# medical-genomics-group/sgVAMP-py

Measured on AMD Instinct MI355X. Metric: VAMP iterations/sec (and effective LD-matvec GB/s) at M markers, K cohorts, higher is better.
Workload: dtype f64

## Files before the change

include/sgvamp_hip.h:

```cpp
#ifndef SGVAMP_HIP_H
#define SGVAMP_HIP_H

#include <stdint.h>

#ifdef __cplusplus
extern "C" {
#endif

#define SGV_OK 0
#define SGV_ERR_HIP (-1)
#define SGV_ERR_ARG (-2)
#define SGV_ERR_RCCL (-3)
#define SGV_ERR_STATE (-4)

#define SGV_ABI_VERSION 2
int sgv_abi_version(void);

#define SGV_MAX_COHORTS 1024
#define SGV_MAX_SLABS 8

#define SGV_VEC_R 0
#define SGV_VEC_R1 1
#define SGV_VEC_XHAT1 2
#define SGV_VEC_XHAT2 3
// ... 132 lines not shown
int sgv_outputs_wait(sgv_ctx* ctx, int slot, double** data);

int sgv_lmmse(sgv_ctx* ctx, int it, const double* gamw, const double* gam2,
              const double* alpha1, const double* alpha2_prev, const int8_t* probes,
              int cg_maxit, double rtol, int lmmse_damp, double rho, int learn_gamw,
              double* out, int* cg_out, int* ld_passes_out);

int sgv_metrics(sgv_ctx* ctx, double* out4);
int sgv_metrics_begin(sgv_ctx* ctx);
int sgv_metrics_end(sgv_ctx* ctx, double* out4);


int sgv_ld_matvec(sgv_ctx* ctx, int ld, int ncol, const double* v, double* y);

int sgv_ld_pass_ex(sgv_ctx* ctx, int ld, int ncol, const double* in, const double* c1,
                   const double* c2, const double* w, uint32_t dot_mask, uint32_t yout_mask,
                   double ys1, double ys0, int run, double* out, double* yout, double* dots);

int sgv_cg_solve(sgv_ctx* ctx, int ld, int ncol, const double* c1, const double* c2,
                 const double* b, double* x, int maxiter, double rtol, int* iters_out,
                 int* info_out);

#define SGV_TIMERS_N 10
int sgv_timers(sgv_ctx* ctx, double* t, int cap, int reset);
#define SGV_EXCHANGE_STATS_N 16
int sgv_exchange_stats(sgv_ctx* ctx, double* out, int cap, int reset);

#define SGV_COMM_INFO_N 5
int sgv_comm_info(sgv_ctx* ctx, int* out, int cap, char* pci_bus_id, int pci_len);

int sgv_exchange_probe(sgv_ctx* ctx, int reps, double* us_out);

int sgv_em_cost_model(double cohort_markers, int nranks, double latency_us, double steps,
                      double* out2);

#define SGV_KIND_NONE 0
#define SGV_KIND_VALU 1
#define SGV_KIND_STRIP4 2
#define SGV_KIND_PAIR 3
#define SGV_KIND_WIDE 4
#define SGV_KIND_STRIP16 5
#define SGV_KIND_WALK 6
#define SGV_PF_KIND 0
#define SGV_PF_VALU_CLASS 1
#define SGV_PF_REST_KIND 2
#define SGV_PF_LOAD_FORM 3
#define SGV_PF_FIN_FORM 4
#define SGV_PF_PK_WIDTH 5
#define SGV_PF_PK_PAIRED 6
#define SGV_PF_DENSE 7
#define SGV_PF_SIDE 8
#define SGV_PF_REST_SIDE 9
#define SGV_PF_MFMA16 10
#define SGV_PF_IDLE_EXIT 11
#define SGV_PF_N 12
int sgv_ld_pass_form(sgv_ctx* ctx, int ld, int ncol, int32_t* form, int cap);

#define SGV_PS_BITS 0
#define SGV_PS_DENSE 1
#define SGV_PS_PACKED 2
#define SGV_PS_WALKS 3
#define SGV_PS_WIDE 4
#define SGV_PS_REST 5
#define SGV_PS_RAGGED 6
#define SGV_PS_PAIR 7
#define SGV_PS_REST_RAGGED 8
#define SGV_PS_REST_PAIR 9
#define SGV_PS_WIDE_IDLE 10
#define SGV_PS_NGRP 11
#define SGV_PS_WIDE_NGRP 12
#define SGV_PS_REST_NGRP 13
#define SGV_PS_N 14
#define SGV_SW_BAND_WALK 0
#define SGV_SW_F32_WALK 1
#define SGV_SW_MF_WIDE 2
#define SGV_SW_MF_PAIR 3
#define SGV_SW_MF_WIDE_IDLE 4
#define SGV_SW_F32_FORM 5
#define SGV_SW_FIN_FORM 6
#define SGV_SW_N 7
int sgv_pass_form_model(const int32_t* shape, const int32_t* switches, int mfma_min, int ncol,
                        int32_t* form, int cap);

int sgv_sync(sgv_ctx* ctx);

int sgv_read_bw(sgv_ctx* ctx, int64_t bytes, int reps, double* gbps);

#ifdef __cplusplus
}
#endif
#endif
```

sgvamp-py_amd/csrc/ctx.h:

```cpp
#pragma once
#include "common.h"
#include "hybrd.h"
#include "../../include/sgvamp_hip.h"

#include <rccl/rccl.h>

#include <algorithm>
#include <atomic>
#include <chrono>
#include <condition_variable>
#include <functional>
#include <mutex>
#include <thread>
#include <limits>
#include <cmath>
#include <cstdarg>
#include <cstdio>
#include <cstdlib>
#include <cstring>
#include <string>
#include <utility>
#include <vector>

using namespace sgv;
// ... 3 lines not shown
  int bits = 64;
  float* f32() const { return reinterpret_cast<float*>(ptr); }
  size_t esz() const { return bits == 32 ? sizeof(float) : sizeof(double); }
  int64_t ext = 0;
  std::vector<int64_t> poff, pw;
  int64_t* d_poff = nullptr;
  int64_t* d_pw = nullptr;
  double stored_bytes = 0.0;
  double stored_elems = 0.0;
};

struct LdCoupling {
  int gb = -1, nr = 0, nc = 0;
  double* d_up = nullptr;
  double* d_lo = nullptr;
};

struct GenoBlock {
  uint32_t* d_bits = nullptr;
  double* d_lut = nullptr;
  double* d_msd = nullptr;
  int64_t stride_w = 0;
  int nsamp = 0;
  int64_t nbad = 0;
};

struct StripSet {
  SymStrip* d_strips = nullptr;
  SymItem* d_sitems = nullptr;
  SymPanel* d_panels = nullptr;
  SymPanelW* d_wpanels = nullptr;
  int nstrips = 0, npanels = 0, nsitems = 0;
  int nslots_items = 0;
  bool ragged = false;
  int pair = 0;
  int ngrp = 1;
  std::vector<int> gs, gp;
};

struct LdPlan {
  bool valid = false;
  int bits = 64;
  RowGroup* d_rg = nullptr;
  int nrg = 0;
  int* d_pbeg = nullptr;
  int nparts = 0;
  SymItem* d_items[4] = {nullptr, nullptr, nullptr, nullptr};
  int nitems[4] = {0, 0, 0, 0};
  SymPanel* d_panels[4] = {nullptr, nullptr, nullptr, nullptr};
  int npanels = 0;
  StripSet s512;
  StripSet wide, rest;
  bool wide_idle = true;
  SymWalk* d_walks = nullptr;
  int nwalks = 0;
  SymPanel* d_wpanels = nullptr;
  SymItem* d_witems = nullptr;
  WalkFin* d_wfins = nullptr;
  int nwfins = 0, nhslots = 0, ncslots = 0;
  double stored_bytes = 0.0, dense_bytes = 0.0;
  double mac_elems = 0.0;
  CouplingTask* d_ctasks = nullptr;
  int nctasks = 0, ncp = 0;
  bool halo = false;
  int64_t hmax = 0, h_src0 = 0, h_src1 = 0;
  int h_len0 = 0, h_len1 = 0;
  double cpl_bytes = 0.0;
};

static inline int mfma_min_default() { return 3; }
static inline int cg_pipe_default() {
  const char* e = ab_env("SGV_CG_PIPE");
  return (e && e[0] == '0') ? 0 : 1;
}
constexpr int CG_RING = 4;
constexpr int MAXGRP = 8;
constexpr int NOUT_SLOTS = 3;

static inline int cg_exact_default() {
  const char* e = ab_env("SGV_CG_EXACT");
  return !e ? -1 : (e[0] == '0' ? 0 : 1);
}
constexpr double CG_EXACT_MIN_BYTES = 24e9;
static inline int sym_class_nc(int cls) { return std::min(16, 2 << (cls + 1)); }

static inline bool fused_ctl_pays(int nv, int nblk) {
  return nblk <= EM_CTL_MAXBLK && nv * nblk <= 128;
}

struct sgv_ctx {
  int dev = 0;
  hipStream_t st = nullptr;
  int K = 0, nld = 0;
  std::vector<int> ld_of;
  int nblk = 0;
  std::vector<int64_t> bn, boff, bvoff;
  int64_t Mloc = 0, Mpad = 0;
  int blk0 = 0, nblk_global = 0;
  int64_t Mtot = 0;
  double s = 0.0;
  std::vector<double> Ncoh;
  std::vector<std::vector<LdBlock>> ldb;
  std::vector<int64_t> lda;
  std::vector<BlkDesc*> d_blks;
  std::vector<LdPlan> plan;
  std::vector<std::vector<LdCoupling>> cpl;
  std::vector<GenoBlock> geno;
  std::vector<int> rank_blk0;
  double* d_cpbuf = nullptr;
  size_t cpbuf_cap = 0;
  double* d_halo = nullptr;
  size_t halo_cap = 0;
  double* h_halo = nullptr;
  size_t h_halo_cap = 0;
  int packing = 1;
  int ld_bits = 64;
  hipStream_t st_fin = nullptr;
  hipEvent_t ev_grp[MAXGRP] = {};
  hipEvent_t ev_fin = nullptr;
  double* d_whead = nullptr;
  double* d_wcarry = nullptr;
  size_t whead_cap = 0, wcarry_cap = 0;
  double* d_rowpart = nullptr;
  double* d_colpart = nullptr;
  size_t rowpart_cap = 0, colpart_cap = 0, part_cap = 0;
  int mfma_min = 3;
  double* d_pk = nullptr;
  double* d_out = nullptr;
  double* h_out[NOUT_SLOTS] = {};
  hipEvent_t ev_out[NOUT_SLOTS] = {};
  int8_t* h_probe[2] = {nullptr, nullptr};
  hipEvent_t ev_probe[2] = {nullptr, nullptr};
  int8_t* d_probe = nullptr;
  std::atomic<size_t> probe_cap{0};
  std::atomic<int> probe_slot{0};
  hipEvent_t ev_unpk[2] = {nullptr, nullptr};
  int pref_slot = -1;
  const int8_t* pref_src = nullptr;
  hipStream_t st_copy = nullptr;
  hipEvent_t ev_pack[NOUT_SLOTS] = {};
  double* h_met = nullptr;
  hipEvent_t ev_met = nullptr;
  int met_pending = 0;
  std::thread worker;
  std::mutex wmu;
  std::condition_variable wcv;
  struct Job {
    std::function<int()> fn;
    std::atomic<int> state{0};
    int rc = 0;
  };
  Job jobs[2];
  uint64_t job_begun = 0, job_ended = 0, job_run = 0;
  std::atomic<bool> worker_quit{false};
  struct Chain {
    int valid = 0;
    std::vector<double> gam1, gamw, alpha1, alpha2;
    double lam, om[MAXL];
  } chain;
  double mle_gam = std::numeric_limits<double>::quiet_NaN();
  double* d_inner = nullptr;
  size_t inner_cap = 0;
  int post_on = 0;
  double post_thr = 0.95;
  double* d_post = nullptr;
  size_t post_cap = 0;
// ... 157 lines not shown
```

sgvamp-py_amd/csrc/ldplan.hip:

```cpp
#include "ctx.h"

void free_plan(LdPlan& p){
  if (p.d_rg) (void)hipFree(p.d_rg);
  if (p.d_pbeg) (void)hipFree(p.d_pbeg);
  for (int k = 0; k < 4; ++k) {
    if (p.d_items[k]) (void)hipFree(p.d_items[k]);
    if (p.d_panels[k]) (void)hipFree(p.d_panels[k]);
  }
  for (StripSet* q : {&p.s512, &p.wide, &p.rest}) {
    if (q->d_strips) (void)hipFree(q->d_strips);
    if (q->d_sitems) (void)hipFree(q->d_sitems);
    if (q->d_panels) (void)hipFree(q->d_panels);
    if (q->d_wpanels) (void)hipFree(q->d_wpanels);
  }
  if (p.d_ctasks) (void)hipFree(p.d_ctasks);
  if (p.d_walks) (void)hipFree(p.d_walks);
  if (p.d_wpanels) (void)hipFree(p.d_wpanels);
  if (p.d_witems) (void)hipFree(p.d_witems);
  if (p.d_wfins) (void)hipFree(p.d_wfins);
  p = LdPlan();
}

void free_block(LdBlock& lb){
  if (lb.ptr) (void)hipFree(lb.ptr);
// ... 2 lines not shown
  lb = LdBlock();
}

static int64_t panel_ext(int64_t n, int64_t r0, int64_t ext) {
  return ext > 0 ? std::min(n - r0, ext) : n - r0;
}

int ld_alloc(sgv_ctx* c, int ld, int b, int fmt, int64_t ext){
  LdBlock& lb = c->ldb[ld][b];
  if (fmt == 0) ext = 0;
  const int bits = fmt == 1 ? c->ld_bits : 64;
  if (lb.ptr && lb.fmt == fmt && lb.ext == ext && lb.bits == bits) return SGV_OK;
  free_block(lb);
  c->plan[ld].valid = false;
  const int64_t n = c->bn[b];
  size_t elems = 0;
  lb.fmt = fmt;
  lb.ext = ext;
  lb.bits = bits;
  if (fmt == 0) {
    elems = (size_t)c->lda[b] * (size_t)n;
    lb.stored_elems = (double)n * (double)n;
    lb.stored_bytes = lb.stored_elems * 8.0;
  } else {
    double valid = 0.0;
    for (int64_t r0 = 0; r0 < n; r0 += SYM_H) {
      const int64_t H = std::min<int64_t>(SYM_H, n - r0);
      const int64_t e = panel_ext(n, r0, ext);
      const int64_t w = round_up(e, PADV);
      lb.poff.push_back((int64_t)elems);
      lb.pw.push_back(w);
      elems += (size_t)(H * w);
      valid += (double)H * (double)e;
    }
    lb.stored_elems = valid;
    lb.stored_bytes = valid * (double)lb.esz();
    HIPCHK(hipMalloc(&lb.d_poff, sizeof(int64_t) * lb.poff.size()));
    HIPCHK(hipMalloc(&lb.d_pw, sizeof(int64_t) * lb.pw.size()));
    HIPCHK(hipMemcpy(lb.d_poff, lb.poff.data(), sizeof(int64_t) * lb.poff.size(),
                     hipMemcpyHostToDevice));
    HIPCHK(hipMemcpy(lb.d_pw, lb.pw.data(), sizeof(int64_t) * lb.pw.size(), hipMemcpyHostToDevice));
  }
  {
    const hipError_t e = hipMalloc(&lb.ptr, lb.esz() * elems);
    if (e != hipSuccess) {
      lb.ptr = nullptr;
      size_t fr = 0, tot = 0;
      (void)hipGetLastError();
      (void)hipMemGetInfo(&fr, &tot);
      return fail(c, SGV_ERR_HIP,
                  "LD matrix %d block %d (n=%lld, %s, %s): %.2f GB of device memory needed, "
                  "%.2f GB free: %s", ld, b, (long long)n,
                  fmt == 0 ? "dense" : ext > 0 ? "packed band" : "packed triangle",
                  bits == 32 ? "f32" : "f64", (double)lb.esz() * (double)elems / 1e9, (double)fr / 1e9,
                  hipGetErrorString(e));
    }
  }
  HIPCHK(hipMemsetAsync(lb.ptr, 0, lb.esz() * elems, c->st));
  BlkDesc d{fmt == 0 ? lb.ptr : nullptr, c->lda[b], c->bn[b], c->bvoff[b]};
  HIPCHK(hipMemcpyAsync(c->d_blks[ld] + b, &d, sizeof d, hipMemcpyHostToDevice, c->st));
  CHK(stream_wait(c));
  return SGV_OK;
}

static int ld_ready(sgv_ctx* c, int ld) {
  for (int b = 0; b < c->nblk; ++b)
    if (!c->ldb[ld][b].ptr)
      return fail(c, SGV_ERR_STATE, "LD matrix %d block %d has not been set", ld, b);
  return SGV_OK;
}

int grow(sgv_ctx* c, double** buf, size_t* cap, size_t need){
  if (need <= *cap) return SGV_OK;
  if (*buf) HIPCHK(hipFree(*buf));
  *buf = nullptr;
  HIPCHK(hipMalloc(buf, sizeof(double) * need));
  *cap = need;
  return SGV_OK;
}


constexpr int MFMA_STRIP = 8;

static int pass_groups(int nstrips, int nblk, int slots) {
  const int g = nstrips / std::max(1, 4 * slots);
  return std::max(1, std::min(std::min(g, 8), nblk));
}

static int device_cus() {
  int dev = 0, ncu = 256;
  if (hipGetDevice(&dev) == hipSuccess) {
    hipDeviceProp_t prop;
    if (hipGetDeviceProperties(&prop, dev) == hipSuccess && prop.multiProcessorCount > 0)
      ncu = prop.multiProcessorCount;
  }
  return ncu;
}

static double lpt_efficiency(std::vector<double> cost, int slots) {
  std::sort(cost.begin(), cost.end(), std::greater<double>());
  std::vector<double> load((size_t)slots, 0.0);
  double tot = 0.0;
  for (double x : cost) {
    auto it = std::min_element(load.begin(), load.end());
    *it += x;
    tot += x;
  }
  const double mk = *std::max_element(load.begin(), load.end());
  return mk > 0.0 ? tot / slots / mk : 1.0;
}

static int mfma_pair_choice(const std::vector<SymStrip>& strips,
                            const std::vector<SymItem>& sitems, int forced) {
  if (forced >= 0) return forced;
  const int ncu = device_cus();
  std::vector<double> cost;
  cost.reserve(strips.size());
  for (const SymStrip& st : strips) {
    double x = 0.0;
    for (int i = 0; i < st.npan; ++i) x += (double)sitems[st.it0 + i].H / SYM_H;
    cost.push_back(x * (double)st.ncmax / 512.0);
  }
  const double quad = lpt_efficiency(cost, 2 * ncu);
  const double pair = lpt_efficiency(cost, ncu);
  return pair >= quad + 0.03 ? 1 : 0;
}

static int build_strips(sgv_ctx* c, int ld, const std::vector<SymItem>& items,
                        const std::vector<SymPanel>& panels, bool wide, int which,
                        int pair_forced, StripSet* out) {
  const int cw = wide ? MFW_CW : 512;
  const int S = MFMA_STRIP;
  const int NPAR = cw / SYM_H;
  auto taken = [&](int b) {
    const LdBlock& lb = c->ldb[ld][b];
    return lb.fmt == 1 && (which == 0 || (which == 1) == (lb.ext == 0));
  };
  std::vector<SymItem> sitems;
  std::vector<SymStrip> strips;
  std::vector<int> sblk;
  std::vector<SymPanelW> sp;
  std::vector<int> pblk;
  int bp0 = 0;
  for (int b = 0; b < c->nblk; ++b) {
    if (c->ldb[ld][b].fmt != 1) continue;
    const int64_t n = c->bn[b];
    const int np = (int)c->ldb[ld][b].poff.size();
    if (!taken(b)) {
      bp0 += np;
      continue;
    }
    const int sp0 = (int)sp.size();
    for (int g = 0; g < np; ++g) {
      SymPanelW w;
      w.p = panels[bp0 + g];
      for (int k = 0; k < 4; ++k) w.sb[k] = w.se[k] = 0;
      sp.push_back(w);
      pblk.push_back(b);
    }
    for (int p = 0; p < NPAR; ++p)
      for (int64_t c0 = (int64_t)SYM_H * p; c0 < n; c0 += cw) {
        const int G = (int)(c0 / SYM_H);
        const int sb = (int)strips.size();
        const int64_t ext = c->ldb[ld][b].ext;
        const int glo = ext > 0 ? std::max(p, G - NPAR * (((int)(ext / SYM_H) - 1) / NPAR)) : p;
        for (int g0 = glo; g0 <= G; g0 += NPAR * S) {
          SymStrip st;
          st.it0 = (int)sitems.size();
          st.npan = 0;
          st.slot = (int)strips.size();
          st.ncmax = 0;
          for (int g = g0; g <= G && g < g0 + NPAR * S; g += NPAR) {
            const SymPanel& pn = panels[bp0 + g];
            const int idx = pn.item_begin + (int)((c0 - (int64_t)SYM_H * g) / cw);
            if (idx >= pn.item_end || items[idx].c0 != c0)
              return fail(c, SGV_ERR_STATE, "strip plan: item (%d, %lld) missing", g,
                          (long long)c0);
            sitems.push_back(items[idx]);
            st.ncmax = std::max(st.ncmax, items[idx].nc);
            ++st.npan;
          }
          strips.push_back(st);
          sblk.push_back(b);
        }
        for (int k = 0; k < NPAR; ++k)
          if (G + k < np) {
            sp[sp0 + G + k].sb[k] = sb;
            sp[sp0 + G + k].se[k] = (int)strips.size();
          }
      }
    bp0 += np;
  }
  *out = StripSet();
  out->nslots_items = (int)items.size();
  if (strips.empty()) return SGV_OK;
  const int ncu = device_cus();
  std::vector<int> grp(c->nblk, 0);
  int ngrp = pass_groups((int)strips.size(), c->nblk, wide ? ncu : 2 * ncu);
  {
    auto bytes = [&](int b) { return which == 0 || taken(b) ? c->ldb[ld][b].stored_bytes : 0.0; };
    double tot = 0.0;
    for (int b = 0; b < c->nblk; ++b) tot += bytes(b);
    double acc = 0.0;
    for (int b = 0; b < c->nblk; ++b) {
      grp[b] = std::min(ngrp - 1, (int)(acc / tot * ngrp));
      acc += bytes(b);
    }
    ngrp = grp[c->nblk - 1] + 1;
  }
  {
    std::vector<int> ord(strips.size());
    for (size_t i = 0; i < ord.size(); ++i) ord[i] = (int)i;
    std::stable_sort(ord.begin(), ord.end(), [&](int x, int y) {
      if (grp[sblk[x]] != grp[sblk[y]]) return grp[sblk[x]] < grp[sblk[y]];
      return strips[x].npan > strips[y].npan;
    });
    std::vector<SymStrip> o(strips.size());
    out->gs.assign(ngrp + 1, 0);
    for (size_t i = 0; i < ord.size(); ++i) {
      o[i] = strips[ord[i]];
      out->gs[grp[sblk[ord[i]]] + 1] = (int)i + 1;
    }
    for (int g = 1; g <= ngrp; ++g) out->gs[g] = std::max(out->gs[g], out->gs[g - 1]);
    strips.swap(o);
  }
  {
    std::vector<int> ord(sp.size());
    for (size_t i = 0; i < ord.size(); ++i) ord[i] = (int)i;
    auto work = [&](const SymPanelW& a) {
      int w = a.p.item_end - a.p.item_begin;
      for (int k = 0; k < 4; ++k) w += a.se[k] - a.sb[k];
      return w;
    };
    std::stable_sort(ord.begin(), ord.end(), [&](int x, int y) {
      if (grp[pblk[x]] != grp[pblk[y]]) return grp[pblk[x]] < grp[pblk[y]];
      return work(sp[x]) > work(sp[y]);
    });
    std::vector<SymPanelW> o(sp.size());
    out->gp.assign(ngrp + 1, 0);
    for (size_t i = 0; i < ord.size(); ++i) {
      o[i] = sp[ord[i]];
      out->gp[grp[pblk[ord[i]]] + 1] = (int)i + 1;
    }
    for (int g = 1; g <= ngrp; ++g) out->gp[g] = std::max(out->gp[g], out->gp[g - 1]);
    sp.swap(o);
  }
  out->ngrp = ngrp;
  out->nstrips = (int)strips.size();
  out->nsitems = (int)sitems.size();
  out->npanels = (int)sp.size();
  out->ragged = false;
  for (const SymStrip& st : strips)
    for (int i = 0; i < st.npan; ++i) out->ragged |= sitems[st.it0 + i].nc < st.ncmax;
  out->pair = (wide || out->ragged) ? 0 : mfma_pair_choice(strips, sitems, pair_forced);
  CHK(upload_table(c, strips, &out->d_strips));
  CHK(upload_table(c, sitems, &out->d_sitems));
  if (wide) {
    CHK(upload_table(c, sp, &out->d_wpanels));
  } else {
    std::vector<SymPanel> p512(sp.size());
    for (size_t i = 0; i < sp.size(); ++i) {
      p512[i] = sp[i].p;
      p512[i].own_sb = sp[i].sb[0];
      p512[i].own_se = sp[i].se[0];
      p512[i].oth_sb = sp[i].sb[1];
      p512[i].oth_se = sp[i].se[1];
    }
    CHK(upload_table(c, p512, &out->d_panels));
  }
  return SGV_OK;
}

static PassSwitches read_pass_switches() {
  auto sw = [](const char* name, char a, char b) {
    const char* e = ab_env(name);
    return e && (e[0] == a || e[0] == b) ? e[0] - '0' : -1;
  };
  PassSwitches s;
  s.band_walk = sw("SGV_BAND_WALK", '0', '0');
  s.f32_walk = sw("SGV_F32_WALK", '1', '1');
  s.mf_wide = sw("SGV_MF_WIDE", '0', '1');
  s.mf_pair = sw("SGV_MF_PAIR", '0', '1');
  s.mf_wide_idle = sw("SGV_MF_WIDE_IDLE", '0', '0');
  s.f32_form = sw("SGV_F32_FORM", '1', '2');
  s.fin_form = sw("SGV_FIN_FORM", '1', '4');
  return s;
}

static int plan_walks(sgv_ctx* c, int ld, const std::vector<SymItem>& items,
                      const std::vector<SymPanel>& panels, LdPlan* pl) {
  bool any = false;
  for (int b = 0; b < c->nblk; ++b) {
// ... 284 lines not shown
  }
  CHK(grow(c, &c->d_rowpart, &c->rowpart_cap, rowpart_need));
  CHK(grow(c, &c->d_colpart, &c->colpart_cap, colpart_need));
  CHK(grow(c, &c->d_part, &c->part_cap, (size_t)nparts * MAXC));
  pl.valid = true;
  return SGV_OK;
}

const int* ld_parts(sgv_ctx* c, int ld){ return c->plan[ld].d_pbeg; }

static int coupling_pass(sgv_ctx* c, const LdPlan& pl, int nc, const PassArgs& pa) {
  const double* recv = nullptr;
  if (pl.halo) {
    const size_t per = 2 * (size_t)nc * pl.hmax;
    double* send = c->d_halo;
    double* drecv = c->d_halo + per;
    HIPCHK(launch_halo_pack(pa, nc, pl.h_src0, pl.h_len0, pl.h_src1, pl.h_len1, pl.hmax, send,
                            c->st));
    CHK(gather_f64(c, send, drecv, per, c->h_halo, c->h_halo ? c->h_halo + per : nullptr));
    recv = drecv;
  }
  if (pl.nctasks)
    HIPCHK(launch_coupling(nc, pl.d_ctasks, pl.nctasks, pa, recv, pl.hmax, c->d_cpbuf, pl.ncp,
                           c->st));
  c->aux_bytes += pl.cpl_bytes + 2.0 * 8.0 * nc * 256.0 * pl.ncp;
  return SGV_OK;
}

static PlanShape plan_shape(const LdPlan& pl) {
  PlanShape ps;
  ps.bits = pl.bits;
  ps.dense = pl.nrg > 0;
  ps.packed = pl.npanels > 0;
  ps.walks = pl.nwalks > 0;
  ps.wide = pl.wide.nstrips > 0;
  ps.rest = pl.rest.nstrips > 0;
  ps.ragged = pl.s512.ragged;
  ps.pair = pl.s512.pair;
  ps.rest_ragged = pl.rest.ragged;
  ps.rest_pair = pl.rest.pair;
  ps.wide_idle = pl.wide_idle;
  ps.ngrp = pl.s512.ngrp;
  ps.wide_ngrp = pl.wide.ngrp;
  ps.rest_ngrp = pl.rest.ngrp;
  return ps;
}

int ld_pass(sgv_ctx* c, int ld, int nc, const PassArgs& pa_in){
  if (nc <= 0) return SGV_OK;
  CHK(ensure_plan(c, ld));
  const LdPlan& pl = c->plan[ld];
  const PassForm f = pass_form(plan_shape(pl), nc, c->mfma_min, read_pass_switches());
  PassArgs pa = pa_in;
  pa.cpbuf = c->d_cpbuf;
  hipEvent_t e0, e1;
  if (c->evpool.size() < 2) {
    HIPCHK(hipEventCreate(&e0));
    HIPCHK(hipEventCreate(&e1));
  } else {
    e0 = c->evpool.back();
    c->evpool.pop_back();
    e1 = c->evpool.back();
    c->evpool.pop_back();
  }
  HIPCHK(hipEventRecord(e0, c->st));
  if (pl.halo || pl.nctasks) CHK(coupling_pass(c, pl, nc, pa));
  if (f.dense) HIPCHK(launch_ld_pass(nc, c->d_blks[ld], pl.d_rg, pl.nrg, pa, c->d_part, c->st));
  if (f.kind == PK_VALU) {
    const int cls = f.valu_class;
    HIPCHK(launch_sym_pass(nc, cls, pl.d_items[cls], pl.nitems[cls], pa, c->d_rowpart,
                           c->d_colpart, c->st));
    HIPCHK(launch_sym_finalize(nc, cls, pl.d_panels[cls], pl.npanels, pa, c->d_rowpart,
                               c->d_colpart, c->d_part, c->st));
    const double cw = (double)(1024 >> cls);
    c->aux_bytes += 2.0 * 8.0 * nc * (double)pl.nitems[cls] * (SYM_H + cw);
  } else if (f.kind != PK_NONE) {
    HIPCHK(launch_pk(pa, nc, c->Mpad, c->d_pk, f.pk_width, f.pk_paired, c->st));
    if (f.kind == PK_WALK) {
      HIPCHK(launch_band_walk(nc, pl.d_walks, pl.nwalks, pl.d_wpanels, pl.d_witems, c->d_pk,
                              f.pk_width, c->Mpad, pa, c->d_whead, c->d_wcarry, pl.d_wfins,
                              pl.nwfins, c->d_part, pl.bits, f.load_form, c->st));
      c->aux_bytes += 2.0 * 8.0 * nc * SYM_H * (double)(pl.nhslots + pl.ncslots);
    } else {
      auto run_set = [&](const StripSet& ss, int kind, bool split, double* rp, double* cp) -> int {
        for (int g = 0; g < ss.ngrp; ++g) {
          const int s0 = ss.gs[g], ns = ss.gs[g + 1] - s0;
          const int p0 = ss.gp[g], npn = ss.gp[g + 1] - p0;
          if (kind == PK_WIDE)
            HIPCHK(launch_sym_mfma_wide(nc, ss.d_strips + s0, ns, ss.d_sitems, pa, c->d_pk, rp,
                                        cp, f.idle_exit, c->st));
          else
            HIPCHK(launch_sym_mfma(nc, ss.d_strips + s0, ns, ss.d_sitems, pa, c->d_pk,
                                   f.pk_width, rp, cp, ss.ragged, kind == PK_PAIR, pl.bits,
                                   f.load_form, c->st));
          hipStream_t fs = c->st;
          if (split) {
            HIPCHK(hipEventRecord(c->ev_grp[g % MAXGRP], c->st));
            HIPCHK(hipStreamWaitEvent(c->st_fin, c->ev_grp[g % MAXGRP], 0));
            fs = c->st_fin;
          }
          if (kind == PK_WIDE)
            HIPCHK(launch_sym_finalize_wide(nc, ss.d_wpanels + p0, npn, pa, rp, cp, c->d_part,
                                            fs));
          else
            HIPCHK(launch_sym_finalize_strip(nc, ss.d_panels + p0, npn, pa, rp, cp, c->d_part,
                                             f.fin_form, fs));
        }
        return SGV_OK;
      };
      if (f.kind == PK_WIDE) {
        CHK(run_set(pl.wide, PK_WIDE, f.side, c->d_rowpart, c->d_colpart));
        if (f.rest_kind != PK_NONE)
          CHK(run_set(pl.rest, f.rest_kind, f.rest_side,
                      c->d_rowpart + (size_t)pl.wide.nslots_items * SYM_H * nc,
                      c->d_colpart + (size_t)pl.wide.nstrips * MFW_CW * nc));
        c->aux_bytes += 2.0 * 8.0 * nc * ((double)pl.wide.nsitems * SYM_H +
                                          (double)pl.wide.nstrips * MFW_CW +
                                          (double)pl.rest.nsitems * SYM_H +
                                          (double)pl.rest.nstrips * 512);
      } else {
        CHK(run_set(pl.s512, f.kind, f.side, c->d_rowpart, c->d_colpart));
        c->aux_bytes += 2.0 * 8.0 * nc * ((double)pl.s512.nsitems * SYM_H +
                                          (double)pl.s512.nstrips * 512);
      }
      if (f.side || f.rest_side) {
        HIPCHK(hipEventRecord(c->ev_fin, c->st_fin));
        HIPCHK(hipStreamWaitEvent(c->st, c->ev_fin, 0));
      }
    }
    c->aux_bytes += 8.0 * (double)c->Mpad * (f.pk_width + nc);
  }
  HIPCHK(hipEventRecord(e1, c->st));
  c->pending.emplace_back(e0, e1);
  c->pending_wide.push_back(f.mfma16 ? 1 : 0);
  c->ld_flops += 2.0 * nc * pl.mac_elems;
  if (f.mfma16) {
    c->ld_flops_wide += 2.0 * nc * pl.mac_elems;
    c->ld_launches_wide += 1.0;
  }
  c->ld_launches += 1.0;
  c->ld_bytes += pl.stored_bytes;
  c->dense_bytes += pl.dense_bytes;
  c->rhs_bytes += 2.0 * nc * (double)c->Mloc * 8.0;
  return SGV_OK;
}

extern "C" int sgv_ld_pass_form(sgv_ctx* c, int ld, int ncol, int32_t* form, int cap) {
  ENTER(c);
  if (ld < 0 || ld >= c->nld || ncol < 1 || ncol > MAXC || !form || cap < 0)
    return fail(c, SGV_ERR_ARG, "sgv_ld_pass_form: bad arguments");
  CHK(ensure_plan(c, ld));
  pass_form_ints(pass_form(plan_shape(c->plan[ld]), ncol, c->mfma_min, read_pass_switches()),
                 form, cap);
  return SGV_OK;
}

static bool host_symmetric(const double* A, int64_t n, int64_t ld) {
  const int64_t T = 64;
  for (int64_t i0 = 0; i0 < n; i0 += T)
    for (int64_t j0 = i0; j0 < n; j0 += T)
      for (int64_t i = i0; i < std::min(n, i0 + T); ++i)
        for (int64_t j = std::max(j0, i + 1); j < std::min(n, j0 + T); ++j)
          if (!(A[i * ld + j] == A[j * ld + i])) return false;
  return true;
}

static bool narrow_f32(const double* src, float* dst, int64_t n) {
  bool ok = true;
  for (int64_t i = 0; i < n; ++i) {
    const float f = (float)src[i];
    ok &= !(std::isinf(f) && std::isfinite(src[i]));
    dst[i] = f;
  }
  return ok;
}

extern "C" int sgv_set_ld_precision(sgv_ctx* c, int bits) {
  ENTER(c);
  if (bits != 64 && bits != 32)
    return fail(c, SGV_ERR_ARG, "sgv_set_ld_precision: %d bits (64 or 32)", bits);
  c->ld_bits = bits;
  return SGV_OK;
}

extern "C" int sgv_ld_block_precision(sgv_ctx* c, int ld, int b, int* bits_out) {
  ENTER(c);
  if (ld < 0 || ld >= c->nld || b < 0 || b >= c->nblk || !bits_out)
    return fail(c, SGV_ERR_ARG, "sgv_ld_block_precision: bad arguments");
  const LdBlock& lb = c->ldb[ld][b];
  *bits_out = lb.ptr ? lb.bits : -1;
  return SGV_OK;
}

extern "C" int sgv_set_ld_packing(sgv_ctx* c, int mode) {
  ENTER(c);
  if (mode != 0 && mode != 1) return fail(c, SGV_ERR_ARG, "packing mode %d", mode);
  c->packing = mode;
  return SGV_OK;
}

extern "C" int sgv_set_ld_block(sgv_ctx* c, int ld, int b, const double* host, int64_t ld_host) {
  ENTER(c);
  if (ld < 0 || ld >= c->nld || b < 0 || b >= c->nblk || !host || ld_host < c->bn[b])
    return fail(c, SGV_ERR_ARG, "sgv_set_ld_block: bad arguments (ld=%d b=%d)", ld, b);
  const int64_t n = c->bn[b];
  const int fmt = (c->packing && host_symmetric(host, n, ld_host)) ? 1 : 0;
  CHK(ld_alloc(c, ld, b, fmt));
  LdBlock& lb = c->ldb[ld][b];
// ... 200 lines not shown
```

sgvamp-py_amd/csrc/pass_form.cpp:

```cpp
#include "pass_form.h"

#include <cstdint>

#include "sgvamp_hip.h"

namespace sgv {

static_assert(PK_NONE == SGV_KIND_NONE && PK_VALU == SGV_KIND_VALU && PK_STRIP4 == SGV_KIND_STRIP4 &&
                  PK_PAIR == SGV_KIND_PAIR && PK_WIDE == SGV_KIND_WIDE &&
                  PK_STRIP16 == SGV_KIND_STRIP16 && PK_WALK == SGV_KIND_WALK,
              "the header names the kinds");

bool plan_wants_walks(int bits, const PassSwitches& sw) {
  return sw.band_walk != 0 && (bits != 32 || sw.f32_walk == 1);
}
static bool walk_pass(const PlanShape& ps, int nc, const PassSwitches& sw) {
  return ps.walks && nc <= 8 && sw.band_walk != 0 &&
         (ps.bits != 32 || (nc >= WALK_F32_MIN_NC && sw.f32_walk == 1));
}

bool plan_wide_idle(const PassSwitches& sw) { return sw.mf_wide_idle != 0; }

int plan_pair_forced(const PassSwitches& sw) {
  return sw.mf_pair < 0 ? -1 : sw.mf_pair == 1 ? 2 : 0;
}

static bool wide_pass(int nc, const PassSwitches& sw) {
  if (nc < 3 || nc > 8) return false;
  if (sw.mf_wide >= 0) return sw.mf_wide == 1;
  return sw.mf_pair < 0;
}

static int strip_kind(int bits, bool ragged, int pair, int nc) {
  if (nc > 8) return PK_STRIP16;
  return bits == 64 && !ragged && pair >= 1 ? PK_PAIR : PK_STRIP4;
}

static int fin_form(bool ragged, int nc, const PassSwitches& sw) {
  return sw.fin_form > 0 ? sw.fin_form : (ragged && nc <= 8) ? 1 : 4;
}

PassForm pass_form(const PlanShape& ps, int nc, int mfma_min, const PassSwitches& sw) {
  PassForm f;
  f.dense = ps.dense;
  if (!ps.packed) return f;
  const bool f32 = ps.bits == 32;
  if (!f32 && !(mfma_min > 0 && nc >= mfma_min)) {
    f.kind = PK_VALU;
    f.valu_class = sym_class(nc);
    return f;
  }
  f.pk_width = nc > 8 ? 16 : nc <= 4 ? 4 : 8;
  f.pk_paired = nc > 4 && nc <= 8;
  const bool walk = walk_pass(ps, nc, sw);
  f.load_form = !f32 ? 1 : sw.f32_form > 0 ? sw.f32_form
                     : walk ? WALK_F32_FORM_DEFAULT : F32_FORM_DEFAULT;
  if (walk) {
    f.kind = PK_WALK;
    return f;
  }
  if (!f32 && ps.wide && wide_pass(nc, sw)) {
    f.kind = PK_WIDE;
    f.idle_exit = ps.wide_idle;
    f.side = ps.wide_ngrp > 1;
    if (ps.rest) {
      f.rest_kind = strip_kind(ps.bits, ps.rest_ragged, ps.rest_pair, nc);
      f.fin_form = fin_form(ps.rest_ragged, nc, sw);
      f.rest_side = ps.rest_ngrp > 1;
    }
    return f;
  }
  f.kind = strip_kind(ps.bits, ps.ragged, ps.pair, nc);
  f.mfma16 = f.kind == PK_STRIP16;
  f.fin_form = fin_form(ps.ragged, nc, sw);
  f.side = ps.ngrp > 1;
  return f;
}

void pass_form_ints(const PassForm& f, int32_t* form, int cap) {
  const int32_t v[SGV_PF_N] = {f.kind, f.valu_class, f.rest_kind, f.load_form, f.fin_form,
                               f.pk_width, f.pk_paired, f.dense, f.side, f.rest_side, f.mfma16,
                               f.idle_exit};
  for (int i = 0; i < cap && i < SGV_PF_N; ++i) form[i] = v[i];
}

}

extern "C" int sgv_pass_form_model(const int32_t* shape, const int32_t* switches, int mfma_min,
                                   int ncol, int32_t* form, int cap) {
  using namespace sgv;
  if (!shape || !switches || !form || cap < 0 || ncol < 1 || ncol > 16) return SGV_ERR_ARG;
  if (shape[SGV_PS_BITS] != 64 && shape[SGV_PS_BITS] != 32) return SGV_ERR_ARG;
  PlanShape ps;
  ps.bits = shape[SGV_PS_BITS];
  ps.dense = shape[SGV_PS_DENSE] != 0;
  ps.packed = shape[SGV_PS_PACKED] != 0;
  ps.walks = shape[SGV_PS_WALKS] != 0;
  ps.wide = shape[SGV_PS_WIDE] != 0;
  ps.rest = shape[SGV_PS_REST] != 0;
  ps.ragged = shape[SGV_PS_RAGGED] != 0;
  ps.pair = shape[SGV_PS_PAIR];
  ps.rest_ragged = shape[SGV_PS_REST_RAGGED] != 0;
  ps.rest_pair = shape[SGV_PS_REST_PAIR];
  ps.wide_idle = shape[SGV_PS_WIDE_IDLE] != 0;
  ps.ngrp = shape[SGV_PS_NGRP];
  ps.wide_ngrp = shape[SGV_PS_WIDE_NGRP];
  ps.rest_ngrp = shape[SGV_PS_REST_NGRP];
  PassSwitches sw;
  sw.band_walk = switches[SGV_SW_BAND_WALK];
  sw.f32_walk = switches[SGV_SW_F32_WALK];
  sw.mf_wide = switches[SGV_SW_MF_WIDE];
  sw.mf_pair = switches[SGV_SW_MF_PAIR];
  sw.mf_wide_idle = switches[SGV_SW_MF_WIDE_IDLE];
  sw.f32_form = switches[SGV_SW_F32_FORM];
  sw.fin_form = switches[SGV_SW_FIN_FORM];
  if ((sw.band_walk != -1 && sw.band_walk != 0) || (sw.f32_walk != -1 && sw.f32_walk != 1) ||
      sw.mf_wide < -1 || sw.mf_wide > 1 || sw.mf_pair < -1 || sw.mf_pair > 1 ||
      (sw.mf_wide_idle != -1 && sw.mf_wide_idle != 0) ||
      (sw.f32_form != -1 && sw.f32_form != 1 && sw.f32_form != 2) ||
      (sw.fin_form != -1 && sw.fin_form != 1 && sw.fin_form != 4))
    return SGV_ERR_ARG;
  pass_form_ints(pass_form(ps, ncol, mfma_min, sw), form, cap);
  return SGV_OK;
}
```

sgvamp-py_amd/csrc/pass_form.h:

```cpp
#pragma once
#include <cstdint>

namespace sgv {

struct PlanShape {
  int bits = 64;
  bool dense = false;
  bool packed = false;
  bool walks = false;
  bool wide = false;
  bool rest = false;
  bool ragged = false;
  int pair = 0;
  bool rest_ragged = false;
  int rest_pair = 0;
  bool wide_idle = true;
  int ngrp = 1, wide_ngrp = 1, rest_ngrp = 1;
};

struct PassSwitches {
  int band_walk = -1;
  int f32_walk = -1;
  int mf_wide = -1;
  int mf_pair = -1;
  int mf_wide_idle = -1;
  int f32_form = -1;
  int fin_form = -1;
};

enum PackedKind {
  PK_NONE = 0,
  PK_VALU = 1,
  PK_STRIP4 = 2,
  PK_PAIR = 3,
  PK_WIDE = 4,
  PK_STRIP16 = 5,
  PK_WALK = 6
};

struct PassForm {
  int kind = PK_NONE;
  int valu_class = -1;
  int rest_kind = PK_NONE;
  int load_form = 0;
  int fin_form = 0;
  int pk_width = 0;
  bool pk_paired = false;
  bool dense = false;
  bool side = false;
  bool rest_side = false;
  bool mfma16 = false;
  bool idle_exit = false;
};

constexpr int F32_FORM_DEFAULT = 2;
constexpr int WALK_F32_FORM_DEFAULT = 2;
constexpr int WALK_F32_MIN_NC = 3;

static inline int sym_class(int nc) { return nc <= 2 ? 0 : nc <= 4 ? 1 : nc <= 8 ? 2 : 3; }

PassForm pass_form(const PlanShape& ps, int nc, int mfma_min, const PassSwitches& sw);

void pass_form_ints(const PassForm& f, int32_t* form, int cap);

bool plan_wants_walks(int bits, const PassSwitches& sw);
bool plan_wide_idle(const PassSwitches& sw);
int plan_pair_forced(const PassSwitches& sw);

}
```

sgvamp-py_amd/hip_backend.py:

```python
import collections
import ctypes
import os

import numpy as np

HERE = os.path.dirname(os.path.abspath(__file__))
LIB_PATH = os.path.join(HERE, "libsgvamp_hip.so")

SGV_OK = 0
VEC_R, VEC_R1, VEC_XHAT1, VEC_XHAT2, VEC_SIG2U, VEC_X0 = range(6)
LMMSE_NOUT = 8
O_TRSIGMA2, O_ALPHA2, O_GAM1, O_Z, O_TRRSIGMA2, O_GAMW, O_XR, O_XRX = range(8)
STEP_EM, STEP_DENOISE_DAMP, STEP_ALPHA1_DAMP, STEP_LMMSE_DAMP, STEP_LEARN_GAMW, STEP_METRICS, \
    STEP_CHAIN, STEP_MLE = 1, 2, 4, 8, 16, 32, 64, 128
STEP_POSTERIOR = 256
POSTERIOR_ROWS = 3
MLE_NOT_CONVERGED, MLE_NEGATIVE = 1, 2
OUT_SLOTS = 3
MAX_COHORTS = 1024
MAX_SLABS = 8
ABI_VERSION = 2
TIMERS_N, EXCHANGE_STATS_N, COMM_INFO_N = 10, 16, 5

PASS_KINDS = ("none", "valu", "strip4", "pair", "wide", "strip16", "walk")
# ... 3 lines not shown
                     "rest_ragged", "rest_pair", "wide_idle", "ngrp", "wide_ngrp", "rest_ngrp")
PASS_SWITCHES = ("SGV_BAND_WALK", "SGV_F32_WALK", "SGV_MF_WIDE", "SGV_MF_PAIR",
                 "SGV_MF_WIDE_IDLE", "SGV_F32_FORM", "SGV_FIN_FORM")
PassForm = collections.namedtuple("PassForm", PASS_FORM_FIELDS)

_c_int_p = ctypes.POINTER(ctypes.c_int)
_c_i64_p = ctypes.POINTER(ctypes.c_int64)
_c_i32_p = ctypes.POINTER(ctypes.c_int32)
_c_dbl_p = ctypes.POINTER(ctypes.c_double)
_c_i8_p = ctypes.POINTER(ctypes.c_int8)
_c_u8_p = ctypes.POINTER(ctypes.c_uint8)
_vp = ctypes.c_void_p

_SIGS = {
    "sgv_create": [ctypes.c_int, ctypes.c_int, ctypes.c_int, _c_int_p, ctypes.c_int, _c_i64_p,
                   ctypes.c_int, ctypes.c_int, ctypes.c_int64, ctypes.POINTER(_vp)],
    "sgv_destroy": [_vp],
    "sgv_last_error": [_vp],
    "sgv_comm_unique_id": [ctypes.c_char_p],
    "sgv_comm_init": [_vp, ctypes.c_int, ctypes.c_int, ctypes.c_char_p, _c_int_p],
    "sgv_comm_init_host": [_vp, ctypes.c_int, ctypes.c_int, _c_int_p, ctypes.c_void_p, _vp],
    "sgv_set_mfma_min": [_vp, ctypes.c_int],
    "sgv_set_cg_pipeline": [_vp, ctypes.c_int],
    "sgv_set_cg_exact": [_vp, ctypes.c_int],
    "sgv_set_rs_recurrence": [_vp, ctypes.c_int],
    "sgv_reset_solver": [_vp],
    "sgv_outputs_begin": [_vp, ctypes.c_int],
    "sgv_outputs_wait": [_vp, ctypes.c_int, ctypes.POINTER(_c_dbl_p)],
    "sgv_mle_exp_max": [_vp, _c_dbl_p, ctypes.c_int, _c_dbl_p, _c_dbl_p],
    "sgv_mle_terms": [_vp, _c_dbl_p, _c_dbl_p, ctypes.c_int, _c_dbl_p, _c_dbl_p, ctypes.c_double,
                      _c_dbl_p],
    "sgv_mle_update": [_vp, _c_dbl_p, _c_dbl_p, ctypes.c_int, _c_dbl_p, _c_dbl_p, _c_dbl_p,
                       _c_dbl_p, _c_int_p],
    "sgv_fsolve": [ctypes.c_int, ctypes.c_void_p, _vp, _c_dbl_p, _c_dbl_p, _c_int_p],
    "sgv_set_mle_gam": [_vp, ctypes.c_double],
    "sgv_set_ld_block": [_vp, ctypes.c_int, ctypes.c_int, _c_dbl_p, ctypes.c_int64],
    "sgv_get_ld_block": [_vp, ctypes.c_int, ctypes.c_int, _c_dbl_p, ctypes.c_int64],
    "sgv_set_ld_block_csr": [_vp, ctypes.c_int, ctypes.c_int, _c_i64_p, _c_i64_p, _c_dbl_p],
    "sgv_set_ld_packing": [_vp, ctypes.c_int],
    "sgv_ld_block_format": [_vp, ctypes.c_int, ctypes.c_int, _c_int_p],
    "sgv_set_ld_precision": [_vp, ctypes.c_int],
    "sgv_ld_block_precision": [_vp, ctypes.c_int, ctypes.c_int, _c_int_p],
    "sgv_ld_stored_bytes": [_vp, ctypes.c_int, _c_dbl_p],
    "sgv_set_ld_coupling": [_vp, ctypes.c_int, ctypes.c_int, ctypes.c_int, ctypes.c_int, _c_dbl_p],
    "sgv_set_ridge": [_vp, ctypes.c_double],
    "sgv_set_cohort_n": [_vp, ctypes.c_int, ctypes.c_double],
    "sgv_set_vector": [_vp, ctypes.c_int, ctypes.c_int, _c_dbl_p],
    "sgv_get_vector": [_vp, ctypes.c_int, ctypes.c_int, _c_dbl_p],
    "sgv_synth_ld_g": [_vp, ctypes.c_int, ctypes.c_uint64, ctypes.c_int64, ctypes.c_int, _c_dbl_p,
                       _c_dbl_p],
    "sgv_synth_r": [_vp, ctypes.c_int, ctypes.c_uint64, ctypes.c_int64, ctypes.c_int, _c_dbl_p],
    "sgv_geno_set_block": [_vp, ctypes.c_int, _c_u8_p, ctypes.c_int64, ctypes.c_int, _c_i64_p],
    "sgv_geno_ld": [_vp, ctypes.c_int, ctypes.c_int],
    "sgv_geno_ld_band": [_vp, ctypes.c_int, ctypes.c_int, ctypes.c_int64],
    "sgv_geno_coupling": [_vp, ctypes.c_int, ctypes.c_int, ctypes.c_int, ctypes.c_int, _c_u8_p,
                          ctypes.c_int64, ctypes.c_int, ctypes.c_int64, _c_i64_p],
    "sgv_geno_ld_band_reach": [_vp, ctypes.c_int, ctypes.c_int, _c_i32_p, _c_dbl_p,
                               ctypes.c_double],
    "sgv_geno_coupling_reach": [_vp, ctypes.c_int, ctypes.c_int, ctypes.c_int, ctypes.c_int,
                                _c_u8_p, ctypes.c_int64, ctypes.c_int, _c_i32_p, _c_dbl_p,
                                ctypes.c_double, _c_i64_p],
    "sgv_geno_r": [_vp, ctypes.c_int, _c_dbl_p],
    "sgv_geno_g": [_vp, _c_dbl_p, _c_dbl_p],
    "sgv_geno_clear": [_vp],
    "sgv_denoise": [_vp, _c_dbl_p, _c_dbl_p, ctypes.c_double, ctypes.c_int, _c_dbl_p, _c_dbl_p,
                    ctypes.c_double, ctypes.c_int, _c_dbl_p],
    "sgv_posterior": [_vp, _c_dbl_p, _c_dbl_p, ctypes.c_double, ctypes.c_int, _c_dbl_p, _c_dbl_p,
                      ctypes.c_double, _c_dbl_p, _c_dbl_p, _c_dbl_p, _c_dbl_p, _c_dbl_p],
    "sgv_set_posterior_outputs": [_vp, ctypes.c_int, ctypes.c_double],
    "sgv_em": [_vp, _c_dbl_p, _c_dbl_p, ctypes.c_int, _c_dbl_p, ctypes.c_int, _c_dbl_p, _c_dbl_p,
               _c_int_p, _c_dbl_p],
    "sgv_lmmse": [_vp, ctypes.c_int, _c_dbl_p, _c_dbl_p, _c_dbl_p, _c_dbl_p, _c_i8_p, ctypes.c_int,
                  ctypes.c_double, ctypes.c_int, ctypes.c_double, ctypes.c_int, _c_dbl_p, _c_int_p,
                  _c_int_p],
    "sgv_metrics": [_vp, _c_dbl_p],
    "sgv_metrics_begin": [_vp],
    "sgv_metrics_end": [_vp, _c_dbl_p],
    "sgv_ld_matvec": [_vp, ctypes.c_int, ctypes.c_int, _c_dbl_p, _c_dbl_p],
    "sgv_ld_pass_ex": [_vp, ctypes.c_int, ctypes.c_int, _c_dbl_p, _c_dbl_p, _c_dbl_p, _c_dbl_p,
                       ctypes.c_uint32, ctypes.c_uint32, ctypes.c_double, ctypes.c_double,
                       ctypes.c_int, _c_dbl_p, _c_dbl_p, _c_dbl_p],
    "sgv_cg_solve": [_vp, ctypes.c_int, ctypes.c_int, _c_dbl_p, _c_dbl_p, _c_dbl_p, _c_dbl_p,
                     ctypes.c_int, ctypes.c_double, _c_int_p, _c_int_p],
    "sgv_abi_version": [],
    "sgv_timers": [_vp, _c_dbl_p, ctypes.c_int, ctypes.c_int],
    "sgv_exchange_stats": [_vp, _c_dbl_p, ctypes.c_int, ctypes.c_int],
    "sgv_comm_info": [_vp, _c_int_p, ctypes.c_int, ctypes.c_char_p, ctypes.c_int],
    "sgv_exchange_probe": [_vp, ctypes.c_int, _c_dbl_p],
    "sgv_em_cost_model": [ctypes.c_double, ctypes.c_int, ctypes.c_double, ctypes.c_double,
                          _c_dbl_p],
    "sgv_step": [_vp, ctypes.c_int, ctypes.c_int, ctypes.c_int, ctypes.c_int, _c_dbl_p, _c_dbl_p,
                 _c_dbl_p, _c_dbl_p, _c_dbl_p, ctypes.c_double, _c_dbl_p, _c_dbl_p, _c_dbl_p,
                 _c_i8_p, ctypes.c_int, ctypes.c_double, ctypes.c_int, _c_dbl_p, _c_int_p,
                 _c_dbl_p, _c_int_p],
    "sgv_step_begin": [_vp, ctypes.c_int, ctypes.c_int, ctypes.c_int, ctypes.c_int, _c_dbl_p,
                       _c_dbl_p, _c_dbl_p, _c_dbl_p, _c_dbl_p, ctypes.c_double, _c_dbl_p,
                       _c_dbl_p, _c_dbl_p, _c_i8_p, ctypes.c_int, ctypes.c_double, ctypes.c_int,
                       _c_dbl_p, _c_int_p, _c_dbl_p, _c_int_p],
    "sgv_step_end": [_vp],
    "sgv_probe_draw": [ctypes.POINTER(ctypes.c_uint32), ctypes.POINTER(ctypes.c_int32),
                       ctypes.c_int64, ctypes.c_int64, ctypes.c_int64, _c_i8_p],
    "sgv_ld_pass_form": [_vp, ctypes.c_int, ctypes.c_int, _c_int_p, ctypes.c_int],
    "sgv_pass_form_model": [_c_int_p, _c_int_p, ctypes.c_int, ctypes.c_int, _c_int_p,
                            ctypes.c_int],
    "sgv_sync": [_vp],
    "sgv_read_bw": [_vp, ctypes.c_int64, ctypes.c_int, _c_dbl_p],
}
_RESTYPES = {"sgv_destroy": None, "sgv_last_error": ctypes.c_char_p}
EXPORTS = tuple(_SIGS)

_lib = None


class HipError(RuntimeError):
    pass


def ab_env(name):
    v = os.environ.get(name)
    if v is None:
        return None
    if os.environ.get("SGV_AB") != "1":
        import warnings

        warnings.warn("%s=%s ignored: A/B overrides need SGV_AB=1" % (name, v))
        return None
    return v


def load(path=LIB_PATH, strict=True):
    global _lib
    if _lib is not None:
        return _lib
    if not os.path.exists(path):
        raise HipError("libsgvamp_hip.so not found at %s -- build it with "
                       "`make -C sgvamp-py_amd/csrc` (there is no CPU fallback)" % path)
    lib = ctypes.CDLL(path)
    for name, args in _SIGS.items():
        if not hasattr(lib, name):
            if not strict:
                continue
            raise HipError("%s does not export %s: stale build -- rebuild with "
                           "`make -C sgvamp-py_amd/csrc`" % (path, name))
        fn = getattr(lib, name)
        fn.argtypes = args
        fn.restype = _RESTYPES.get(name, ctypes.c_int)
    if strict and lib.sgv_abi_version() != ABI_VERSION:
        raise HipError("%s has ABI version %d, this binding expects %d: rebuild with "
                       "`make -C sgvamp-py_amd/csrc`" % (path, lib.sgv_abi_version(), ABI_VERSION))
    _lib = lib
    return lib


def pass_form_of(ints):
    v = [int(x) for x in ints]
    named = {"kind": PASS_KINDS[v[0]], "rest_kind": PASS_KINDS[v[2]]}
    flags = ("pk_paired", "dense", "side", "rest_side", "mfma16", "idle_exit")
    return PassForm(*[named.get(f, bool(x) if f in flags else x)
                      for f, x in zip(PASS_FORM_FIELDS, v)])


def pass_form_model(shape, switches, mfma_min, ncol):
    dflt = {"bits": 64, "wide_idle": 1, "ngrp": 1, "wide_ngrp": 1, "rest_ngrp": 1}
    assert set(shape) <= set(PLAN_SHAPE_FIELDS) and set(switches) <= set(PASS_SWITCHES)
    sh = np.array([int(shape.get(f, dflt.get(f, 0))) for f in PLAN_SHAPE_FIELDS], dtype=np.int32)
    sw = np.array([int(switches.get(n, -1)) for n in PASS_SWITCHES], dtype=np.int32)
# ... 142 lines not shown
```

Baseline: 30.38.

## Run closing strip group's finalize on main stream with tail-sized group plan

Replaces the fixed byte-balanced strip grouping with a planner that, by default, reserves a closing group sized to about one wave of slots and balances the leading blocks into the remaining groups. The final group's finalize then runs on the main stream instead of the side stream, and the side stream is joined before it, which removes a trailing cross-stream event wait. The goal is to shrink the serialized tail where the last finalize waits on the side stream. In exchange there are fewer or unevenly sized groups and less overlap for the last group. The behaviour can be switched off with SGV_PASS_EDGES=0.

Result: no change. 30.27 (-0.3%).

```diff
diff --git a/include/sgvamp_hip.h b/include/sgvamp_hip.h
--- a/include/sgvamp_hip.h
+++ b/include/sgvamp_hip.h
@@ -238,6 +238,9 @@
 int sgv_pass_form_model(const int32_t* shape, const int32_t* switches, int mfma_min, int ncol,
                         int32_t* form, int cap);
 
+int sgv_pass_groups_model(const int32_t* blk_strips, const double* blk_w, int nblk, int slots,
+                          int closing, int32_t* grp, int32_t* ngrp_out);
+
 int sgv_sync(sgv_ctx* ctx);
 
 int sgv_read_bw(sgv_ctx* ctx, int64_t bytes, int reps, double* gbps);
diff --git a/sgvamp-py_amd/csrc/ctx.h b/sgvamp-py_amd/csrc/ctx.h
--- a/sgvamp-py_amd/csrc/ctx.h
+++ b/sgvamp-py_amd/csrc/ctx.h
@@ -109,6 +109,10 @@
   return !e ? -1 : (e[0] == '0' ? 0 : 1);
 }
 constexpr double CG_EXACT_MIN_BYTES = 24e9;
+static inline bool pass_edges() {
+  const char* e = ab_env("SGV_PASS_EDGES");
+  return !(e && e[0] == '0' && !e[1]);
+}
 static inline int sym_class_nc(int cls) { return std::min(16, 2 << (cls + 1)); }
 
 static inline bool fused_ctl_pays(int nv, int nblk) {
diff --git a/sgvamp-py_amd/csrc/ldplan.hip b/sgvamp-py_amd/csrc/ldplan.hip
--- a/sgvamp-py_amd/csrc/ldplan.hip
+++ b/sgvamp-py_amd/csrc/ldplan.hip
@@ -108,10 +108,7 @@
 
 constexpr int MFMA_STRIP = 8;
 
-static int pass_groups(int nstrips, int nblk, int slots) {
-  const int g = nstrips / std::max(1, 4 * slots);
-  return std::max(1, std::min(std::min(g, 8), nblk));
-}
+static_assert(PASS_MAXGRP == MAXGRP, "one event per group");
 
 static int device_cus() {
   int dev = 0, ncu = 256;
@@ -221,19 +218,13 @@
   out->nslots_items = (int)items.size();
   if (strips.empty()) return SGV_OK;
   const int ncu = device_cus();
-  std::vector<int> grp(c->nblk, 0);
-  int ngrp = pass_groups((int)strips.size(), c->nblk, wide ? ncu : 2 * ncu);
-  {
-    auto bytes = [&](int b) { return which == 0 || taken(b) ? c->ldb[ld][b].stored_bytes : 0.0; };
-    double tot = 0.0;
-    for (int b = 0; b < c->nblk; ++b) tot += bytes(b);
-    double acc = 0.0;
-    for (int b = 0; b < c->nblk; ++b) {
-      grp[b] = std::min(ngrp - 1, (int)(acc / tot * ngrp));
-      acc += bytes(b);
-    }
-    ngrp = grp[c->nblk - 1] + 1;
-  }
+  std::vector<int32_t> grp(c->nblk, 0), bstrips(c->nblk, 0);
+  std::vector<double> bw(c->nblk, 0.0);
+  for (int b : sblk) ++bstrips[b];
+  for (int b = 0; b < c->nblk; ++b)
+    bw[b] = which == 0 || taken(b) ? c->ldb[ld][b].stored_bytes : 0.0;
+  const int ngrp = pass_group_plan(bstrips.data(), bw.data(), c->nblk, wide ? ncu : 2 * ncu,
+                                   pass_edges(), grp.data());
   {
     std::vector<int> ord(strips.size());
     for (size_t i = 0; i < ord.size(); ++i) ord[i] = (int)i;
@@ -684,7 +675,10 @@
                               pl.nwfins, c->d_part, pl.bits, f.load_form, c->st));
       c->aux_bytes += 2.0 * 8.0 * nc * SYM_H * (double)(pl.nhslots + pl.ncslots);
     } else {
-      auto run_set = [&](const StripSet& ss, int kind, bool split, double* rp, double* cp) -> int {
+      bool side_open = false;
+      const bool tail_main = pass_edges();
+      auto run_set = [&](const StripSet& ss, int kind, bool split, double* rp, double* cp,
+                         bool last_set) -> int {
         for (int g = 0; g < ss.ngrp; ++g) {
           const int s0 = ss.gs[g], ns = ss.gs[g + 1] - s0;
           const int p0 = ss.gp[g], npn = ss.gp[g + 1] - p0;
@@ -696,10 +690,17 @@
                                    f.pk_width, rp, cp, ss.ragged, kind == PK_PAIR, pl.bits,
                                    f.load_form, c->st));
           hipStream_t fs = c->st;
-          if (split) {
+          if (split && last_set && g == ss.ngrp - 1 && tail_main) {
+            if (side_open) {
+              HIPCHK(hipEventRecord(c->ev_fin, c->st_fin));
+              HIPCHK(hipStreamWaitEvent(c->st, c->ev_fin, 0));
+              side_open = false;
+            }
+          } else if (split) {
             HIPCHK(hipEventRecord(c->ev_grp[g % MAXGRP], c->st));
             HIPCHK(hipStreamWaitEvent(c->st_fin, c->ev_grp[g % MAXGRP], 0));
             fs = c->st_fin;
+            side_open = true;
           }
           if (kind == PK_WIDE)
             HIPCHK(launch_sym_finalize_wide(nc, ss.d_wpanels + p0, npn, pa, rp, cp, c->d_part,
@@ -711,21 +712,21 @@
         return SGV_OK;
       };
       if (f.kind == PK_WIDE) {
-        CHK(run_set(pl.wide, PK_WIDE, f.side, c->d_rowpart, c->d_colpart));
+        CHK(run_set(pl.wide, PK_WIDE, f.side, c->d_rowpart, c->d_colpart, f.rest_kind == PK_NONE));
         if (f.rest_kind != PK_NONE)
           CHK(run_set(pl.rest, f.rest_kind, f.rest_side,
                       c->d_rowpart + (size_t)pl.wide.nslots_items * SYM_H * nc,
-                      c->d_colpart + (size_t)pl.wide.nstrips * MFW_CW * nc));
+                      c->d_colpart + (size_t)pl.wide.nstrips * MFW_CW * nc, true));
         c->aux_bytes += 2.0 * 8.0 * nc * ((double)pl.wide.nsitems * SYM_H +
                                           (double)pl.wide.nstrips * MFW_CW +
                                           (double)pl.rest.nsitems * SYM_H +
                                           (double)pl.rest.nstrips * 512);
       } else {
-        CHK(run_set(pl.s512, f.kind, f.side, c->d_rowpart, c->d_colpart));
+        CHK(run_set(pl.s512, f.kind, f.side, c->d_rowpart, c->d_colpart, true));
         c->aux_bytes += 2.0 * 8.0 * nc * ((double)pl.s512.nsitems * SYM_H +
                                           (double)pl.s512.nstrips * 512);
       }
-      if (f.side || f.rest_side) {
+      if (side_open) {
         HIPCHK(hipEventRecord(c->ev_fin, c->st_fin));
         HIPCHK(hipStreamWaitEvent(c->st, c->ev_fin, 0));
       }
diff --git a/sgvamp-py_amd/csrc/pass_form.cpp b/sgvamp-py_amd/csrc/pass_form.cpp
--- a/sgvamp-py_amd/csrc/pass_form.cpp
+++ b/sgvamp-py_amd/csrc/pass_form.cpp
@@ -1,6 +1,8 @@
 #include "pass_form.h"
 
+#include <algorithm>
 #include <cstdint>
+#include <vector>
 
 #include "sgvamp_hip.h"
 
@@ -77,6 +79,55 @@
   return f;
 }
 
+static int balance_groups(const double* w, int nb, int n, int32_t* grp) {
+  double tot = 0.0, acc = 0.0;
+  for (int b = 0; b < nb; ++b) tot += w[b];
+  for (int b = 0; b < nb; ++b) {
+    grp[b] = std::min(n - 1, (int)(acc / tot * n));
+    acc += w[b];
+  }
+  return grp[nb - 1] + 1;
+}
+
+int pass_group_plan(const int32_t* blk_strips, const double* blk_w, int nblk, int slots,
+                    bool closing, int32_t* grp) {
+  int64_t nstrips = 0;
+  for (int b = 0; b < nblk; ++b) nstrips += blk_strips[b];
+  const int64_t g = nstrips / std::max(1, 4 * slots);
+  const int n0 = (int)std::max<int64_t>(1, std::min<int64_t>(std::min<int64_t>(g, PASS_MAXGRP), nblk));
+  if (!closing) return balance_groups(blk_w, nblk, n0, grp);
+  for (int b = 0; b < nblk; ++b) grp[b] = 0;
+  if (n0 <= 1) return 1;
+  int e = nblk;
+  int64_t cs = 0;
+  while (e > 1 && cs < slots) cs += blk_strips[--e];
+  double wlead = 0.0;
+  for (int b = 0; b < e; ++b) wlead += blk_w[b];
+  if (!(wlead > 0.0)) return 1;
+  std::vector<int32_t> lab((size_t)e);
+  for (int n = n0 - 1; n >= 1; --n) {
+    balance_groups(blk_w, e, n, lab.data());
+    int ng = 1;
+    int64_t least = -1, cur = 0;
+    for (int b = 0; b < e; ++b) {
+      if (b > 0 && lab[b] != lab[b - 1]) {
+        if (least < 0 || cur < least) least = cur;
+        cur = 0;
+        ++ng;
+      }
+      cur += blk_strips[b];
+      grp[b] = ng - 1;
+    }
+    if (least < 0 || cur < least) least = cur;
+    if (least >= cs) {
+      for (int b = e; b < nblk; ++b) grp[b] = ng;
+      return ng + 1;
+    }
+  }
+  for (int b = 0; b < nblk; ++b) grp[b] = 0;
+  return 1;
+}
+
 void pass_form_ints(const PassForm& f, int32_t* form, int cap) {
   const int32_t v[SGV_PF_N] = {f.kind, f.valu_class, f.rest_kind, f.load_form, f.fin_form,
                                f.pk_width, f.pk_paired, f.dense, f.side, f.rest_side, f.mfma16,
@@ -123,3 +174,18 @@
   pass_form_ints(pass_form(ps, ncol, mfma_min, sw), form, cap);
   return SGV_OK;
 }
+
+extern "C" int sgv_pass_groups_model(const int32_t* blk_strips, const double* blk_w, int nblk,
+                                     int slots, int closing, int32_t* grp, int32_t* ngrp_out) {
+  if (!blk_strips || !blk_w || !grp || !ngrp_out || nblk < 1 || slots < 1 ||
+      (closing != 0 && closing != 1))
+    return SGV_ERR_ARG;
+  double tot = 0.0;
+  for (int b = 0; b < nblk; ++b) {
+    if (blk_strips[b] < 0 || !(blk_w[b] >= 0.0)) return SGV_ERR_ARG;
+    tot += blk_w[b];
+  }
+  if (!(tot > 0.0)) return SGV_ERR_ARG;
+  *ngrp_out = sgv::pass_group_plan(blk_strips, blk_w, nblk, slots, closing != 0, grp);
+  return SGV_OK;
+}
diff --git a/sgvamp-py_amd/csrc/pass_form.h b/sgvamp-py_amd/csrc/pass_form.h
--- a/sgvamp-py_amd/csrc/pass_form.h
+++ b/sgvamp-py_amd/csrc/pass_form.h
@@ -63,6 +63,10 @@
 
 void pass_form_ints(const PassForm& f, int32_t* form, int cap);
 
+constexpr int PASS_MAXGRP = 8;
+int pass_group_plan(const int32_t* blk_strips, const double* blk_w, int nblk, int slots,
+                    bool closing, int32_t* grp);
+
 bool plan_wants_walks(int bits, const PassSwitches& sw);
 bool plan_wide_idle(const PassSwitches& sw);
 int plan_pair_forced(const PassSwitches& sw);
diff --git a/sgvamp-py_amd/hip_backend.py b/sgvamp-py_amd/hip_backend.py
--- a/sgvamp-py_amd/hip_backend.py
+++ b/sgvamp-py_amd/hip_backend.py
@@ -109,6 +109,8 @@
                        ctypes.c_int, _c_dbl_p, _c_dbl_p, _c_dbl_p],
     "sgv_cg_solve": [_vp, ctypes.c_int, ctypes.c_int, _c_dbl_p, _c_dbl_p, _c_dbl_p, _c_dbl_p,
                      ctypes.c_int, ctypes.c_double, _c_int_p, _c_int_p],
+    "sgv_pass_groups_model": [_c_i32_p, _c_dbl_p, ctypes.c_int, ctypes.c_int, ctypes.c_int,
+                              _c_i32_p, _c_i32_p],
     "sgv_abi_version": [],
     "sgv_timers": [_vp, _c_dbl_p, ctypes.c_int, ctypes.c_int],
     "sgv_exchange_stats": [_vp, _c_dbl_p, ctypes.c_int, ctypes.c_int],
```
